# fusioninfer/fusioninfer

Hardware: NVIDIA H100
Metric: routing decisions/sec (4K-tok prompts x 1024 endpoints); achieved HBM GB/s (higher is better)
Workload: dtype u64

## Files before the change

### fusioninfer_b200/csrc/bitslice.cuh

```cuda
#pragma once
#include <stdint.h>

#include "xxh64.cuh"

namespace fi {

constexpr int NPLANES = 10;

struct BitCounter {
  uint32_t c[NPLANES];
};

FI_HD void bc_clear(BitCounter& b) {
#pragma unroll
  for (int i = 0; i < NPLANES; ++i) b.c[i] = 0;
}

template <int LVL>
FI_HD void bc_ripple(BitCounter& b, uint32_t e) {
#pragma unroll
  for (int pl = LVL; pl < NPLANES; ++pl) {
    uint32_t t = b.c[pl] & e;
    b.c[pl] ^= e;
    e = t;
// ... 27 lines not shown
      w[i] = (a & x) | (a & y) | (x & y);
    }
  }
  if (K >= 16) {
    uint32_t a = b.c[3], x = w[0], y = w[1 % K];
    b.c[3] = a ^ x ^ y;
    w[0] = (a & x) | (a & y) | (x & y);
  }
  if (K == 1) bc_ripple<0>(b, w[0]);
  if (K == 2) bc_ripple<1>(b, w[0]);
  if (K == 4) bc_ripple<2>(b, w[0]);
  if (K == 8) bc_ripple<3>(b, w[0]);
  if (K == 16) bc_ripple<4>(b, w[0]);
}

FI_HD void bc_merge(BitCounter& b, const BitCounter& o) {
  uint32_t carry = 0;
#pragma unroll
  for (int pl = 0; pl < NPLANES; ++pl) {
    uint32_t x = b.c[pl], y = o.c[pl];
    b.c[pl] = x ^ y ^ carry;
    carry = (x & y) | (x & carry) | (y & carry);
  }
}

FI_HD uint32_t bc_nonzero(const BitCounter& b) {
  uint32_t m = 0;
#pragma unroll
  for (int pl = 0; pl < NPLANES; ++pl) m |= b.c[pl];
  return m;
// ... 11 lines not shown
```

### fusioninfer_b200/csrc/engine.cu

```cuda
#include <cuda_runtime.h>
#include <unistd.h>
#include <dlfcn.h>

#include <algorithm>
#include <atomic>
#include <chrono>
#include <cmath>
#include <condition_variable>
#include <cstdio>
#include <cstdlib>
#include <cstring>
#include <functional>
#include <memory>
#include <mutex>
#include <string>
#include <thread>
#include <unordered_set>
#include <vector>

#include <sched.h>

#include "../../include/fi_epp.h"
#include "kernels.cuh"
#include "lru.h"
// ... 303 lines not shown
      }
    }
    h->ev_pool.push_back(e.a);
    h->ev_pool.push_back(e.b);
  }
  h->pending_ev.clear();
}

void free_index(IndexView& v) {
  cudaFree(v.keys);
  cudaFree(v.node_of);
  cudaFree(v.klog);
  cudaFree(v.rows);
  cudaFree(v.cnt);
  cudaFree(v.rmask);
  v.keys = nullptr;
  v.node_of = nullptr;
  v.klog = nullptr;
  v.rows = nullptr;
  v.cnt = nullptr;
  v.rmask = nullptr;
}

size_t index_bytes(uint64_t slots, uint32_t W) {
  const uint64_t total = slots + 3;
  return total * (sizeof(uint64_t) * 2 + sizeof(uint32_t) * 3 + (size_t)W * sizeof(uint32_t));
}

int clear_index(fi_epp* h, IndexView& v) {
  const uint64_t total = v.C + 3;
  FI_CUDA(cudaMemsetAsync(v.keys, 0, total * sizeof(uint64_t), h->s_index));
  FI_CUDA(cudaMemsetAsync(v.node_of, 0xFF, total * sizeof(uint32_t), h->s_index));
  FI_CUDA(cudaMemsetAsync(v.klog, 0, total * sizeof(uint64_t), h->s_index));
  FI_CUDA(cudaMemsetAsync(v.rows, 0, total * v.W * sizeof(uint32_t), h->s_index));
  FI_CUDA(cudaMemsetAsync(v.cnt, 0, total * sizeof(uint32_t), h->s_index));
  FI_CUDA(cudaMemsetAsync(v.rmask, 0, total * sizeof(uint32_t), h->s_index));
  return FI_OK;
}

int alloc_index(fi_epp* h, uint64_t slots, IndexView* out) {
  IndexView v{};
  v.C = slots;
  v.bmask = slots / BUCKET_KEYS - 1;
  v.W = h->W;
  v.logW = 0;
  while ((1u << v.logW) < v.W) ++v.logW;
  const uint64_t total = slots + 3;
  size_t free_b = 0, total_b = 0;
  if (cudaMemGetInfo(&free_b, &total_b) == cudaSuccess && index_bytes(slots, v.W) + (256ull << 20) > free_b) {
    h->err = "index of " + std::to_string(index_bytes(slots, v.W) >> 20) + " MiB does not fit in the " +
             std::to_string(free_b >> 20) + " MiB of free device memory";
    return FI_ERR_NOMEM;
  }
  cudaError_t e = cudaMalloc(&v.keys, total * sizeof(uint64_t));
  if (e == cudaSuccess) e = cudaMalloc(&v.node_of, total * sizeof(uint32_t));
  if (e == cudaSuccess) e = cudaMalloc(&v.klog, total * sizeof(uint64_t));
  if (e == cudaSuccess) e = cudaMalloc(&v.rows, total * v.W * sizeof(uint32_t));
  if (e == cudaSuccess) e = cudaMalloc(&v.cnt, total * sizeof(uint32_t));
  if (e == cudaSuccess) e = cudaMalloc(&v.rmask, total * sizeof(uint32_t));
  if (e != cudaSuccess) {
    cudaGetLastError();
    free_index(v);
    h->err = std::string("index allocation: ") + cudaGetErrorString(e);
    return e == cudaErrorMemoryAllocation ? FI_ERR_NOMEM : FI_ERR_CUDA;
  }
  int rc = clear_index(h, v);
  if (rc != FI_OK) {
    free_index(v);
    return rc;
  }
  *out = v;
  return FI_OK;
}

// ... 2308 lines not shown
  drain_profile(h);
  h->profiling = on != 0;
  return FI_OK;
}

int fi_epp_get_stats(fi_epp* h, fi_epp_stats* out) {
  if (!h || !out) return FI_ERR_INVALID;
  std::lock_guard<std::mutex> lk(h->mu);
  if (cudaSetDevice(h->cfg.device) != cudaSuccess) return fail(h, FI_ERR_CUDA, "cudaSetDevice failed");
  drain_profile(h);
  if (h->profiling) {
    FI_CUDA(cudaStreamSynchronize(h->s_main));
    unsigned long long pb[8] = {0};
    FI_CUDA(cudaMemcpy(pb, h->d_probed, sizeof(pb), cudaMemcpyDeviceToHost));
    h->stats.probed_blocks = pb[0];
    if (pb[5] && h->verbose)
      std::fprintf(stderr, "[fi_epp] match_pick phases, cycles per request over %llu requests: stage %.0f, first lookup %.0f, "
                   "chunks %.0f, score+pick %.0f\n", pb[5], (double)pb[1] / pb[5], (double)pb[2] / pb[5], (double)pb[3] / pb[5],
                   (double)pb[4] / pb[5]);
  }
  *out = h->stats;
  return FI_OK;
}

int fi_epp_reset_stats(fi_epp* h) {
  if (!h) return FI_ERR_INVALID;
  std::lock_guard<std::mutex> lk(h->mu);
  cudaSetDevice(h->cfg.device);
  drain_profile(h);
  cudaStreamSynchronize(h->s_main);
// ... 7 lines not shown
```

### fusioninfer_b200/csrc/hostcheck.cpp

```cpp
#include <cstdint>
#include <cstring>
#include <algorithm>
#include <set>
#include <unordered_map>
#include <unordered_set>
#include <vector>

#include "bitslice.cuh"
#include "lru.h"
#include "lru_batch.h"
#include "lru_plan.h"
#include "tiebreak.cuh"
#include "xxh64.cuh"

extern "C" {

uint64_t fihc_xxh64(const uint8_t* p, uint32_t len) { return fi::xxh64_bytes(p, len); }

uint32_t fihc_chain_generic(const uint8_t* p, uint64_t len, uint64_t h0, uint32_t B, uint32_t M, uint64_t* out) {
  uint64_t nb = len / B;
  if (nb > M) nb = M;
  uint64_t h = h0;
  for (uint64_t i = 0; i < nb; ++i) {
    fi::ChainMsg m{p + i * B, B, h, true};
// ... 25 lines not shown
void fihc_bitcount(const uint32_t* words, uint32_t n, uint32_t K, uint32_t* counts) {
  fi::BitCounter b;
  fi::bc_clear(b);
  for (uint32_t i = 0; i < n; i += K) {
    uint32_t w[16] = {0};
    for (uint32_t j = 0; j < K && i + j < n; ++j) w[j] = words[i + j];
    switch (K) {
      case 1: { uint32_t t[1] = {w[0]}; fi::bc_add<1>(b, t); break; }
      case 2: { uint32_t t[2] = {w[0], w[1]}; fi::bc_add<2>(b, t); break; }
      case 4: { uint32_t t[4]; std::memcpy(t, w, sizeof(t)); fi::bc_add<4>(b, t); break; }
      case 8: { uint32_t t[8]; std::memcpy(t, w, sizeof(t)); fi::bc_add<8>(b, t); break; }
      default: { uint32_t t[16]; std::memcpy(t, w, sizeof(t)); fi::bc_add<16>(b, t); break; }
    }
  }
  for (uint32_t bit = 0; bit < 32; ++bit) counts[bit] = fi::bc_get(b, bit);
}

void fihc_bitcount_merge(const uint32_t* wa, uint32_t na, const uint32_t* wb, uint32_t nb, uint32_t* counts,
                         uint32_t* nonzero) {
  fi::BitCounter a, b;
  fi::bc_clear(a);
  fi::bc_clear(b);
  for (uint32_t i = 0; i < na; ++i) { uint32_t t[1] = {wa[i]}; fi::bc_add<1>(a, t); }
  for (uint32_t i = 0; i < nb; ++i) { uint32_t t[1] = {wb[i]}; fi::bc_add<1>(b, t); }
  fi::bc_merge(a, b);
  for (uint32_t bit = 0; bit < 32; ++bit) counts[bit] = fi::bc_get(a, bit);
  *nonzero = fi::bc_nonzero(a);
}

uint32_t fihc_tie_start(uint32_t n_blocks, uint64_t first_hash, uint64_t h0, uint32_t r, uint32_t E) {
// ... 200 lines not shown
```

### fusioninfer_b200/csrc/index_kernels.cu

```cuda
#include "index_device.cuh"
#include "kernels.cuh"

namespace fi {

namespace {

__device__ uint32_t table_find_or_claim(const IndexView& ix, IndexCounters* ctr, uint64_t h, bool* claimed) {
  *claimed = false;
  uint64_t b = h & ix.bmask;
  for (uint64_t it = 0; it <= ix.bmask; ++it) {
    unsigned long long* kb = reinterpret_cast<unsigned long long*>(ix.keys + b * BUCKET_KEYS);
#pragma unroll 1
    for (int j = 0; j < BUCKET_KEYS; ++j) {
      unsigned long long k = *reinterpret_cast<volatile unsigned long long*>(kb + j);
      if (k == h) return (uint32_t)(b * BUCKET_KEYS + j);
      if (k == KEY_EMPTY) {
        unsigned long long old = atomicCAS(kb + j, (unsigned long long)KEY_EMPTY, (unsigned long long)h);
        if (old == KEY_EMPTY) {
          *claimed = true;
          return (uint32_t)(b * BUCKET_KEYS + j);
        }
        if (old == h) return (uint32_t)(b * BUCKET_KEYS + j);
      }
    }
// ... 19 lines not shown
      tot += c;
    }
    s_base = tot ? atomicAdd(counter, (unsigned long long)tot) : 0ull;
  }
  __syncthreads();
  const unsigned long long pos = flag ? s_base + s_warp[warp] + rank_in_warp : ~0ull;
  __syncthreads();
  return pos;
}

__device__ __forceinline__ uint32_t wait_node(const IndexView& ix, uint32_t slot) {
  const volatile uint32_t* p = ix.node_of + slot;
  uint32_t n;
  while ((n = *p) == NODE_INVALID) __nanosleep(20);
  return n;
}

template <bool REMOTE>
__global__ void __launch_bounds__(256) index_set_kernel(IndexView ix, IndexCounters* ctr, const fi_index_op* __restrict__ ops,
                                                        const uint64_t* __restrict__ hashes, uint64_t n, uint32_t ep_begin,
                                                        uint32_t ep_count, uint32_t rank, GossipLog log) {
  const uint32_t rbit = 1u << rank;
  const uint32_t zero_node = (uint32_t)(ix.C + 2);
  for (uint64_t base = blockIdx.x * (uint64_t)blockDim.x; base < n; base += (uint64_t)gridDim.x * blockDim.x) {
    const uint64_t i = base + threadIdx.x;
    uint64_t hsh = 0;
    bool active = false;
    uint32_t e = 0;
    if (i < n) {
      if (REMOTE) {
// ... 22 lines not shown
      } else {
        atomicExch(&ctr->overflow, 1ull);
        ix.keys[slot] = KEY_TOMB;
        __threadfence();
        *reinterpret_cast<volatile uint32_t*>(ix.node_of + slot) = zero_node;
      }
    }
    if (active && !claimed && slot != SLOT_MISS) node = wait_node(ix, slot);
    bool appear = false;
    if (active && node != NODE_INVALID && node != zero_node) {
      if (REMOTE) {
        atomicOr(ix.rmask + node, rbit);
      } else {
        const uint32_t bit = 1u << (e & 31);
        const uint32_t old = atomicOr(ix.rows + ((uint64_t)node << ix.logW) + (e >> 5), bit);
        if (!(old & bit) && atomicAdd(ix.cnt + node, 1u) == 0u) {
          atomicOr(ix.rmask + node, rbit);
          appear = true;
        }
      }
    }
    if (!REMOTE && log.n_appear) {
      const unsigned long long pos = cta_reserve(appear, log.n_appear);
      if (appear && pos < log.cap) log.appear[pos] = hsh;
    }
  }
}

__device__ uint32_t table_find_slot(const IndexView& ix, uint64_t h) {
  uint64_t b = h & ix.bmask;
// ... 46 lines not shown
    uint32_t slot = SLOT_MISS, node;
    if (key_is_special(hsh)) {
      node = (uint32_t)(ix.C + (hsh == KEY_TOMB ? 1 : 0));
    } else {
      slot = table_find_slot(ix, hsh);
      if (slot == SLOT_MISS) continue;
      node = ix.node_of[slot];
      if (node >= ix.C) continue;
    }
    if (REMOTE) {
      rank_vanished(ix, ctr, slot, node, rbit);
      continue;
    }
    const uint32_t bit = 1u << (e & 31);
    const uint32_t old = atomicAnd(ix.rows + ((uint64_t)node << ix.logW) + (e >> 5), ~bit);
    if ((old & bit) && atomicSub(ix.cnt + node, 1u) == 1u) {
      rank_vanished(ix, ctr, slot, node, rbit);
      if (log.n_vanish) {
        const unsigned long long pos = atomicAdd(log.n_vanish, 1ull);
        if (pos < log.cap) log.vanish[pos] = hsh;
      }
    }
  }
}

__global__ void __launch_bounds__(256) index_rebuild_kernel(IndexView from, IndexView to, IndexCounters* ctr) {
  for (uint64_t base = blockIdx.x * (uint64_t)blockDim.x; base < from.C; base += (uint64_t)gridDim.x * blockDim.x) {
    const uint64_t s = base + threadIdx.x;
    uint64_t h = 0;
    if (s < from.C) h = from.klog[s];
    bool claimed = false;
    uint32_t slot = SLOT_MISS;
    if (h != 0) slot = table_find_or_claim(to, ctr, h, &claimed);
    const unsigned long long d = cta_reserve(claimed, &ctr->used);
    if (claimed && d < to.C) {
      to.klog[d] = h;
      to.node_of[slot] = (uint32_t)d;
      to.cnt[d] = from.cnt[s];
      to.rmask[d] = from.rmask[s];
      const uint32_t* src = from.rows + (s << from.logW);
      uint32_t* dst = to.rows + (d << to.logW);
      for (uint32_t w = 0; w < from.W; ++w) dst[w] = src[w];
    }
  }
  if (blockIdx.x == 0 && threadIdx.x < 2) {
    const uint64_t s = from.C + threadIdx.x;
    if (from.rmask[s]) {
      to.cnt[s] = from.cnt[s];
      to.rmask[s] = from.rmask[s];
      for (uint32_t w = 0; w < from.W; ++w) to.rows[(s << to.logW) + w] = from.rows[(s << from.logW) + w];
    }
  }
}


__device__ __forceinline__ uint32_t sweep_node(const IndexView& ix, uint64_t t, uint64_t n) {
  return (uint32_t)(t < n ? t : ix.C + (t - n));
}
// ... 104 lines not shown
      if (node != SLOT_MISS) r = (ix.rows[((uint64_t)node << ix.logW) + (e >> 5)] >> (e & 31)) & 1u;
    }
    out[i] = r;
  }
}

inline unsigned grid_for(uint64_t n) {
  uint64_t g = (n + 255) / 256;
  if (g > 132ull * 16) g = 132ull * 16;
  if (g == 0) g = 1;
  return (unsigned)g;
}

}

cudaError_t launch_index_set(IndexView ix, IndexCounters* ctr, const fi_index_op* ops, uint64_t n, uint32_t ep_begin,
                             uint32_t ep_count, uint32_t rank, GossipLog log, cudaStream_t s) {
  if (n == 0) return cudaSuccess;
  index_set_kernel<false><<<grid_for(n), 256, 0, s>>>(ix, ctr, ops, nullptr, n, ep_begin, ep_count, rank, log);
  return cudaGetLastError();
}

cudaError_t launch_index_clear(IndexView ix, IndexCounters* ctr, const fi_index_op* ops, uint64_t n,
                               uint32_t ep_begin, uint32_t ep_count, uint32_t rank, GossipLog log, cudaStream_t s) {
  if (n == 0) return cudaSuccess;
  index_clear_kernel<false><<<grid_for(n), 256, 0, s>>>(ix, ctr, ops, nullptr, n, ep_begin, ep_count, rank, log, nullptr);
  return cudaGetLastError();
}

cudaError_t launch_index_clear_counted(IndexView ix, IndexCounters* ctr, const fi_index_op* ops, uint64_t cap,
                                       const unsigned long long* n_dev, uint32_t ep_begin, uint32_t ep_count, uint32_t rank,
                                       GossipLog log, cudaStream_t s) {
  if (cap == 0) return cudaSuccess;
  index_clear_kernel<false><<<grid_for(cap), 256, 0, s>>>(ix, ctr, ops, nullptr, cap, ep_begin, ep_count, rank, log, n_dev);
  return cudaGetLastError();
}

cudaError_t launch_index_remote_appear(IndexView ix, IndexCounters* ctr, const uint64_t* hashes, uint64_t n, uint32_t rank,
                                       cudaStream_t s) {
  if (n == 0) return cudaSuccess;
  index_set_kernel<true><<<grid_for(n), 256, 0, s>>>(ix, ctr, nullptr, hashes, n, 0, 0, rank, GossipLog{});
  return cudaGetLastError();
}

cudaError_t launch_index_remote_vanish(IndexView ix, IndexCounters* ctr, const uint64_t* hashes, uint64_t n, uint32_t rank,
                                       cudaStream_t s) {
  if (n == 0) return cudaSuccess;
  index_clear_kernel<true><<<grid_for(n), 256, 0, s>>>(ix, ctr, nullptr, hashes, n, 0, 0, rank, GossipLog{}, nullptr);
  return cudaGetLastError();
}
// ... 26 lines not shown
```

### fusioninfer_b200/csrc/kernels.cuh

```cuda
#pragma once
#include <cuda_runtime.h>
#include <stdint.h>

#include "../../include/fi_epp.h"

namespace fi {

constexpr uint32_t SLOT_MISS = 0xFFFFFFFFu;
constexpr uint64_t KEY_EMPTY = 0ull;
constexpr uint64_t KEY_TOMB = ~0ull;
constexpr int BUCKET_KEYS = 4;

struct IndexView {
  uint64_t* keys;
  uint32_t* node_of;
  uint64_t* klog;
  uint32_t* rows;
  uint32_t* cnt;
  uint32_t* rmask;
  uint64_t bmask;
  uint64_t C;
  uint32_t W;
  uint32_t logW;
};

struct IndexCounters {
  unsigned long long used;
  unsigned long long tombstones;
  unsigned long long overflow;
  unsigned long long pad;
};

struct GossipLog {
  unsigned long long* n_appear;
// ... 162 lines not shown
```

### fusioninfer_b200/csrc/match_kernels.cu

```cuda
#include <climits>

#include "bitslice.cuh"
#include "index_device.cuh"
#include "kernels.cuh"
#include "tiebreak.cuh"

namespace fi {

namespace {

constexpr int kWarps = 8;
#ifndef FI_MATCH_MIN_BLOCKS
#define FI_MATCH_MIN_BLOCKS 2
#endif
constexpr unsigned FULL = 0xFFFFFFFFu;

struct Best {
  double score;
  uint32_t e;
  uint32_t m;
  uint32_t k;
};

struct TieRot {
  uint32_t start;
  uint32_t E;
// ... 39 lines not shown
      else if (pr.kind[s] == FI_SCORER_LORA)
        v = lora_v;
      else if (REQ_QUEUE && pr.kind[s] == FI_SCORER_QUEUE)
        v = q_v;
      else
        v = sc_p[(uint64_t)s * Epad + e];
      total = __dadd_rn(total, __dmul_rn(v, pr.weight[s]));
    }
  }
  return total;
}

__device__ __forceinline__ void cp_async16(void* smem, const void* gmem) {
  unsigned sa = (unsigned)__cvta_generic_to_shared(smem);
  asm volatile("cp.async.cg.shared.global [%0], [%1], 16;\n" ::"r"(sa), "l"(gmem));
}
__device__ __forceinline__ void cp_async_wait_all() { asm volatile("cp.async.wait_all;\n" ::: "memory"); }
__device__ __forceinline__ void ll_store(uint64_t* p, uint32_t data, uint32_t tag) {
  asm volatile("st.relaxed.sys.global.u64 [%0], %1;\n" ::"l"(p), "l"(((uint64_t)tag << 32) | data) : "memory");
}
__device__ __forceinline__ uint64_t ll_load(const uint64_t* p) {
  uint64_t v;
  asm volatile("ld.relaxed.sys.global.u64 %0, [%1];\n" : "=l"(v) : "l"(p) : "memory");
  return v;
}
constexpr long long kPollTimeoutCycles = 20000000000ll;
__device__ __forceinline__ bool pd_prefill_runs(uint32_t dec_endpoint, uint32_t dec_match, uint32_t n, uint64_t len,
                                                double threshold) {
  double hit = (dec_endpoint != FI_NO_ENDPOINT && n) ? __ddiv_rn((double)dec_match, (double)n) : 0.0;
  double miss_bytes = __dmul_rn(__dsub_rn(1.0, hit), (double)len);
// ... 10 lines not shown
    out[2 % VEC] = v.z;
    out[3 % VEC] = v.w;
  } else if (VEC == 2) {
    uint2 v = make_uint2(0, 0);
    if (ok) v = __ldg(reinterpret_cast<const uint2*>(p));
    out[0] = v.x;
    out[1 % VEC] = v.y;
  } else {
    out[0] = ok ? __ldg(p) : 0u;
  }
}

constexpr int kSpecTries = 4;
constexpr int kSpecChunks = 8;

__device__ __forceinline__ uint32_t resolve_request_nodes(const IndexView& ix, const uint64_t* __restrict__ s_chain,
                                                          uint32_t* __restrict__ s_node, uint32_t n, int lane, bool have_first,
                                                          uint32_t first_node) {
  uint32_t pos = 0;
  for (int tries = 0; pos < n; ++tries) {
    if (tries < kSpecTries) {
      uint32_t nf = SLOT_MISS;
      if (tries == 0 && have_first) {
        nf = first_node;
      } else {
        if (lane == 0) nf = index_find(ix, s_chain[pos]);
        nf = __shfl_sync(FULL, nf, 0);
      }
      if (nf == SLOT_MISS) return pos;
      if (lane == 0) s_node[pos] = nf;
      uint32_t fail = n;
      if (nf >= ix.C) {
        fail = pos + 1;
      } else {
        for (uint32_t i0 = pos + 1; i0 < n && fail == n; i0 += 32 * kSpecChunks) {
          uint64_t hk[kSpecChunks], kk[kSpecChunks];
#pragma unroll
          for (int c = 0; c < kSpecChunks; ++c) {
            const uint32_t idx = i0 + 32 * c + lane;
            hk[c] = 0;
            kk[c] = 1;
            if (idx < n) {
              hk[c] = s_chain[idx];
              const uint64_t cand = (uint64_t)nf + (idx - pos);
              if (cand < ix.C) kk[c] = __ldg(ix.klog + cand);
            }
          }
#pragma unroll
          for (int c = 0; c < kSpecChunks; ++c) {
            const uint32_t idx = i0 + 32 * c + lane;
            if (fail != n || i0 + 32 * c >= n) break;
            const bool ok = idx < n && kk[c] == hk[c] && !key_is_special(hk[c]);
            const unsigned bad = __ballot_sync(FULL, idx < n && !ok);
            const uint32_t upto = bad ? (uint32_t)(__ffs(bad) - 1) : 32u;
            if ((uint32_t)lane < upto && idx < n) s_node[idx] = nf + (idx - pos);
            if (bad) fail = i0 + 32 * c + upto;
          }
        }
      }
      pos = fail;
    } else {
      const uint32_t ia = pos + lane, ib = pos + 32 + lane;
      uint32_t na = SLOT_MISS, nb = SLOT_MISS;
      if (ia < n) na = index_find_lazy(ix, s_chain[ia]);
      if (ib < n) nb = index_find_lazy(ix, s_chain[ib]);
      const unsigned ma = __ballot_sync(FULL, ia < n && na == SLOT_MISS);
      const unsigned mb = __ballot_sync(FULL, ib < n && nb == SLOT_MISS);
      const uint32_t upto = ma ? (uint32_t)(__ffs(ma) - 1) : (mb ? 32u + (uint32_t)(__ffs(mb) - 1) : 64u);
      if ((uint32_t)lane < upto && ia < n) s_node[ia] = na;
      if ((uint32_t)lane + 32 < upto && ib < n) s_node[ib] = nb;
      if (ma || mb) return pos + upto;
      pos = pos + 64 < n ? pos + 64 : n;
    }
  }
  return n;
}

__device__ __forceinline__ uint32_t take_ticket(uint32_t* counter, uint32_t opaque_zero) {
  uint32_t t;
  asm volatile("atom.relaxed.gpu.global.add.u32 %0, [%1], 1;\n" : "=r"(t) : "l"(counter + opaque_zero) : "memory");
  return t;
}

template <int VEC, int G, bool SUBSET>
__device__ __forceinline__ void ranked_profile(const MatchParams& p, uint32_t pi, const BitCounter (&cnt)[VEC],
                                               const uint32_t (&sub)[VEC], const TieRot& tr, uint32_t n, uint32_t r,
                                               int lane, int t, int g, uint32_t& dec_e, uint32_t& dec_m) {
  const ProfileDev& pr = p.st.prof[pi];
  const double* sc_p = p.st.sc + (uint64_t)pi * FI_EPP_MAX_SCORERS * p.st.Epad;
  const bool lora = p.st.has_lora != 0;
// ... 105 lines not shown
__global__ void __launch_bounds__(kWarps * 32, (VEC >= 4 || RANKED ? FI_MATCH_MIN_BLOCKS : FI_MATCH_MIN_BLOCKS + 1))
    match_pick_kernel(const MatchParams p) {
  constexpr int G = 32 / LPR;
#ifndef FI_MATCH_BATCH
#define FI_MATCH_BATCH 16
#endif
  constexpr int BATCH_MAX = (LPM || VEC >= 4) ? 8 : FI_MATCH_BATCH;
  constexpr int BATCH = LPR < BATCH_MAX ? LPR : BATCH_MAX;
  extern __shared__ __align__(16) uint64_t s_mem[];
  const int warp = threadIdx.x >> 5;
  const int lane = threadIdx.x & 31;
  const int t = lane % LPR;
  const int g = lane / LPR;
  uint64_t* const s_chain_base = s_mem + (size_t)(2 * warp) * p.MP;
  uint32_t* s_node = reinterpret_cast<uint32_t*>(s_mem + (size_t)2 * kWarps * p.MP) + (size_t)warp * p.MP;
  const IndexView ix = p.ix;
  const uint32_t P = p.st.n_profiles;
  const char* row_base = reinterpret_cast<const char*>(ix.rows + t * VEC);
  const uint32_t row_bytes = 4u << ix.logW;
  const uint32_t zero_slot = (uint32_t)(ix.C + 2);

  const uint32_t row_units = p.MP / 2;
  auto stage = [&](uint32_t rr, uint64_t* dst) {
    const uint64_t* crow = p.chain + (uint64_t)rr * p.MP;
    for (uint32_t u = lane; u < row_units; u += 32) cp_async16(dst + 2 * u, crow + 2 * u);
  };
  uint32_t r_next = 0;
  if (lane == 0) r_next = take_ticket(p.work_counter, threadIdx.x & p.lane_zero);
  r_next = __shfl_sync(FULL, r_next, 0);
  int buf = 0;
  if (r_next < p.R) stage(r_next, s_chain_base);
  bool pf_ok = false;
  uint64_t pf_h = 0, pf_key = 0;
  uint32_t pf_node = 0;
  for (;;) {
    const uint32_t r = r_next;
    if (r >= p.R) break;
    if (lane == 0) r_next = take_ticket(p.work_counter, threadIdx.x & p.lane_zero);
    const uint32_t n = p.nblocks[r];
    uint32_t sub[VEC];
#pragma unroll
    for (int x = 0; x < VEC; ++x) {
      sub[x] = 0u;
      if constexpr (SUBSET) {
        const uint32_t wi = t * VEC + x;
        if (wi < p.sub_pitch) sub[x] = __ldg(p.subsets + (uint64_t)r * p.sub_pitch + wi);
      }
    }
    uint64_t* s_chain = s_chain_base + (size_t)buf * p.MP;
#ifdef FI_MATCH_TIMING
    const long long tm0 = clock64();
#endif
    cp_async_wait_all();
    __syncwarp();
    bool have_first = false;
    uint32_t first_node = SLOT_MISS;
    if (pf_ok && n) {
      const unsigned hit = __ballot_sync(FULL, lane < BUCKET_KEYS && pf_key == pf_h);
      const unsigned emp = __ballot_sync(FULL, lane < BUCKET_KEYS && pf_key == KEY_EMPTY);
      if (hit) {
        first_node = __shfl_sync(FULL, pf_node, __ffs(hit) - 1);
        have_first = true;
      } else if (emp) {
        have_first = true;
      }
    }

#ifdef FI_MATCH_TIMING
    const long long tm1 = clock64();
#endif
    BitCounter cnt[VEC];
    uint32_t alive[VEC];
#pragma unroll
    for (int x = 0; x < VEC; ++x) {
      bc_clear(cnt[x]);
      alive[x] = 0xFFFFFFFFu;
    }
    uint32_t matched_rows = 0;
    bool real_miss = false;

    const uint32_t m_rows = resolve_request_nodes(ix, s_chain, s_node, n, lane, have_first, first_node);
    real_miss = m_rows < n;
    __syncwarp();
    r_next = __shfl_sync(FULL, r_next, 0);
    pf_ok = false;
    if (r_next < p.R) {
      stage(r_next, s_chain_base + (size_t)(buf ^ 1) * p.MP);
      pf_h = __ldg(p.chain + (uint64_t)r_next * p.MP);
    }
#ifdef FI_MATCH_TIMING
    const long long tm2 = clock64();
#endif
#pragma unroll 1
    for (uint32_t b0 = 0; b0 < m_rows; b0 += BATCH * G) {
      uint32_t w[VEC][BATCH];
#pragma unroll
      for (int qi = 0; qi < BATCH; ++qi) {
        const uint32_t j = b0 + qi * G + g;
        const uint32_t sn = j < m_rows ? s_node[j] : zero_slot;
        uint32_t tmp[VEC];
        load_row_words<VEC>(reinterpret_cast<const uint32_t*>(row_base + (uint64_t)sn * row_bytes), true, tmp);
#pragma unroll
        for (int x = 0; x < VEC; ++x) w[x][qi] = tmp[x];
      }
      if (LPM) {
#pragma unroll
        for (int qi = 0; qi < BATCH; ++qi) {
#pragma unroll
          for (int x = 0; x < VEC; ++x) {
            uint32_t v = w[x][qi];
            if (G > 1) {
#pragma unroll
              for (int d = 1; d < G; d <<= 1) {
                const uint32_t o = __shfl_up_sync(FULL, v, d * LPR);
                if (g >= d) v &= o;
              }
              v &= alive[x];
              alive[x] = __shfl_sync(FULL, v, (G - 1) * LPR + t);
            } else {
              v &= alive[x];
              alive[x] = v;
            }
            w[x][qi] = v;
          }
        }
      }
#pragma unroll
      for (int x = 0; x < VEC; ++x) {
        uint32_t any = 0;
#pragma unroll
        for (int qi = 0; qi < BATCH; ++qi) any |= w[x][qi];
        if (__any_sync(FULL, any != 0)) bc_add<BATCH>(cnt[x], w[x]);
      }
      matched_rows = min(m_rows, b0 + BATCH * G);
      if (LPM) {
        bool any = false;
#pragma unroll
        for (int x = 0; x < VEC; ++x) any |= alive[x] != 0;
        if (!__ballot_sync(FULL, any)) break;
      }
    }

    if (r_next < p.R && !key_is_special(pf_h)) {
      pf_ok = true;
      if (lane < BUCKET_KEYS) {
        const uint64_t slot0 = (pf_h & ix.bmask) * BUCKET_KEYS + lane;
        pf_key = __ldg(ix.keys + slot0);
        pf_node = __ldg(ix.node_of + slot0);
      }
    }
#ifdef FI_MATCH_TIMING
    const long long tm3 = clock64();
#endif
    const bool nothing = matched_rows == 0;
    if (G > 1 && !nothing) {
#pragma unroll
      for (int x = 0; x < VEC; ++x) {
#pragma unroll
        for (int d = LPR; d < 32; d <<= 1) {
          BitCounter o;
#pragma unroll
          for (int pl = 0; pl < NPLANES; ++pl) o.c[pl] = __shfl_xor_sync(FULL, cnt[x].c[pl], d);
          bc_merge(cnt[x], o);
// ... 123 lines not shown
      if (p.apply_pd) {
        const uint64_t len = p.offsets[r + 1] - p.offsets[r];
        if (!pd_prefill_runs(dec_e, dec_m, n, len, p.pd_threshold)) {
          fi_pick pk;
          pk.endpoint = FI_NO_ENDPOINT;
          pk.match_blocks = 0;
          pk.n_blocks = (uint16_t)n;
          pk.score = 0.0;
          if constexpr (RANKED) {
            for (uint32_t j = 0; j < p.k; ++j) p.out[((uint64_t)r * P + p.pd_prefill) * p.k + j] = pk;
          } else {
            p.out[(uint64_t)r * P + p.pd_prefill] = pk;
          }
        }
      }
      if (p.probed_blocks) atomicAdd(p.probed_blocks, (unsigned long long)(matched_rows + (real_miss ? 1 : 0)));
#ifdef FI_MATCH_TIMING
      if (p.probed_blocks) {
        const long long tm4 = clock64();
        atomicAdd(p.probed_blocks + 1, (unsigned long long)(tm1 - tm0));
        atomicAdd(p.probed_blocks + 2, (unsigned long long)(tm2 - tm1));
        atomicAdd(p.probed_blocks + 3, (unsigned long long)(tm3 - tm2));
        atomicAdd(p.probed_blocks + 4, (unsigned long long)(tm4 - tm3));
        atomicAdd(p.probed_blocks + 5, 1ull);
      }
#endif
    }
    buf ^= 1;
    __syncwarp();
  }
}
// ... 154 lines not shown
    __syncthreads();
    const double zbest = s_best;
    for (uint32_t e = tid; e < st.Epad; e += blockDim.x) {
      bool ok;
      const double tot = zero_total(e, &ok, false);
      const unsigned word = __ballot_sync(FULL, ok && tot == zbest);
      if (lane == 0) ztie[(uint64_t)pi * W + e / 32] = word;
    }
    __syncthreads();
  }
}

template <int LPR, int VEC, bool LPM, bool LORA, bool RANKED, bool SUBSET = false>
cudaError_t launch_match_variant(const MatchParams& p, int sm_count, cudaStream_t s) {
  const auto kern = match_pick_kernel<LPR, VEC, LPM, LORA, RANKED, SUBSET>;
  const size_t smem = (size_t)kWarps * p.MP * (2 * sizeof(uint64_t) + sizeof(uint32_t));
  static size_t cached_smem_dev[64];
  static int cached_per_sm_dev[64];
  int dev = 0;
  cudaError_t e = cudaGetDevice(&dev);
  if (e != cudaSuccess) return e;
  dev &= 63;
  size_t& cached_smem = cached_smem_dev[dev];
  int& cached_per_sm = cached_per_sm_dev[dev];
  if (cached_smem != smem + 1) {
    if (smem > 48 * 1024) {
      e = cudaFuncSetAttribute(kern, cudaFuncAttributeMaxDynamicSharedMemorySize, (int)smem);
      if (e != cudaSuccess) return e;
    }
    int per_sm = 0;
    e = cudaOccupancyMaxActiveBlocksPerMultiprocessor(&per_sm, kern, kWarps * 32, smem);
// ... 62 lines not shown
```

Before: 90.29 million.

## Skip identical consecutive index rows using a same-as-previous bitmap in match

Adds a per-slot bitmap recording whether an index row equals the previous slot's row, maintained by dirty-list fixup kernels after index set/clear and carried through rebuild. The match kernel compresses each request's matched chain into run heads and adds each distinct row once with a run-length bit-sliced add, instead of reading every row. The aim is to cut HBM row traffic for long prefix chains. The first-bucket prefetch also moves to shared memory through cp.async. In exchange, index updates get extra atomics and a fixup kernel launch, and the match path gets more branching and shared-memory bookkeeping.

```diff
diff --git a/fusioninfer_b200/csrc/bitslice.cuh b/fusioninfer_b200/csrc/bitslice.cuh
--- a/fusioninfer_b200/csrc/bitslice.cuh
+++ b/fusioninfer_b200/csrc/bitslice.cuh
@@ -65,6 +65,16 @@
   if (K == 16) bc_ripple<4>(b, w[0]);
 }
 
+FI_HD void bc_add_run(BitCounter& b, uint32_t L, uint32_t w) {
+  uint32_t carry = 0;
+#pragma unroll
+  for (int pl = 0; pl < NPLANES; ++pl) {
+    const uint32_t x = b.c[pl], y = w & (0u - ((L >> pl) & 1u));
+    b.c[pl] = x ^ y ^ carry;
+    carry = (x & y) | (x & carry) | (y & carry);
+  }
+}
+
 FI_HD void bc_merge(BitCounter& b, const BitCounter& o) {
   uint32_t carry = 0;
 #pragma unroll
diff --git a/fusioninfer_b200/csrc/engine.cu b/fusioninfer_b200/csrc/engine.cu
--- a/fusioninfer_b200/csrc/engine.cu
+++ b/fusioninfer_b200/csrc/engine.cu
@@ -341,17 +341,28 @@
   cudaFree(v.rows);
   cudaFree(v.cnt);
   cudaFree(v.rmask);
+  cudaFree(v.same);
+  cudaFree(v.dirty);
+  cudaFree(v.n_dirty);
   v.keys = nullptr;
   v.node_of = nullptr;
   v.klog = nullptr;
   v.rows = nullptr;
   v.cnt = nullptr;
   v.rmask = nullptr;
-}
+  v.same = nullptr;
+  v.dirty = nullptr;
+  v.n_dirty = nullptr;
+}
+
+constexpr uint64_t kDirtyCap = kOpChunk;
+
+uint64_t same_words(uint64_t slots) { return slots / 32 + 1; }
 
 size_t index_bytes(uint64_t slots, uint32_t W) {
   const uint64_t total = slots + 3;
-  return total * (sizeof(uint64_t) * 2 + sizeof(uint32_t) * 3 + (size_t)W * sizeof(uint32_t));
+  return total * (sizeof(uint64_t) * 2 + sizeof(uint32_t) * 3 + (size_t)W * sizeof(uint32_t)) +
+         same_words(slots) * sizeof(uint32_t) + kDirtyCap * sizeof(uint32_t) + sizeof(unsigned long long);
 }
 
 int clear_index(fi_epp* h, IndexView& v) {
@@ -362,6 +373,8 @@
   FI_CUDA(cudaMemsetAsync(v.rows, 0, total * v.W * sizeof(uint32_t), h->s_index));
   FI_CUDA(cudaMemsetAsync(v.cnt, 0, total * sizeof(uint32_t), h->s_index));
   FI_CUDA(cudaMemsetAsync(v.rmask, 0, total * sizeof(uint32_t), h->s_index));
+  FI_CUDA(cudaMemsetAsync(v.same, 0, same_words(v.C) * sizeof(uint32_t), h->s_index));
+  FI_CUDA(cudaMemsetAsync(v.n_dirty, 0, sizeof(unsigned long long), h->s_index));
   return FI_OK;
 }
 
@@ -385,6 +398,10 @@
   if (e == cudaSuccess) e = cudaMalloc(&v.rows, total * v.W * sizeof(uint32_t));
   if (e == cudaSuccess) e = cudaMalloc(&v.cnt, total * sizeof(uint32_t));
   if (e == cudaSuccess) e = cudaMalloc(&v.rmask, total * sizeof(uint32_t));
+  if (e == cudaSuccess) e = cudaMalloc(&v.same, same_words(slots) * sizeof(uint32_t));
+  if (e == cudaSuccess) e = cudaMalloc(&v.dirty, kDirtyCap * sizeof(uint32_t));
+  if (e == cudaSuccess) e = cudaMalloc(&v.n_dirty, sizeof(unsigned long long));
+  v.dirty_cap = kDirtyCap;
   if (e != cudaSuccess) {
     cudaGetLastError();
     free_index(v);
@@ -2723,6 +2740,8 @@
     unsigned long long pb[8] = {0};
     FI_CUDA(cudaMemcpy(pb, h->d_probed, sizeof(pb), cudaMemcpyDeviceToHost));
     h->stats.probed_blocks = pb[0];
+    if (h->verbose && pb[0])
+      std::fprintf(stderr, "[fi_epp] match_pick rows read %llu for %llu blocks probed\n", pb[6], pb[0]);
     if (pb[5] && h->verbose)
       std::fprintf(stderr, "[fi_epp] match_pick phases, cycles per request over %llu requests: stage %.0f, first lookup %.0f, "
                    "chunks %.0f, score+pick %.0f\n", pb[5], (double)pb[1] / pb[5], (double)pb[2] / pb[5], (double)pb[3] / pb[5],
diff --git a/fusioninfer_b200/csrc/hostcheck.cpp b/fusioninfer_b200/csrc/hostcheck.cpp
--- a/fusioninfer_b200/csrc/hostcheck.cpp
+++ b/fusioninfer_b200/csrc/hostcheck.cpp
@@ -63,6 +63,17 @@
     }
   }
   for (uint32_t bit = 0; bit < 32; ++bit) counts[bit] = fi::bc_get(b, bit);
+}
+
+void fihc_bitcount_run(const uint32_t* planes, uint32_t L, uint32_t w, uint32_t* run_out, uint32_t* rep_out) {
+  fi::BitCounter a, b;
+  for (int pl = 0; pl < fi::NPLANES; ++pl) a.c[pl] = b.c[pl] = planes[pl];
+  fi::bc_add_run(a, L, w);
+  for (uint32_t i = 0; i < L; ++i) { uint32_t t[1] = {w}; fi::bc_add<1>(b, t); }
+  for (int pl = 0; pl < fi::NPLANES; ++pl) {
+    run_out[pl] = a.c[pl];
+    rep_out[pl] = b.c[pl];
+  }
 }
 
 void fihc_bitcount_merge(const uint32_t* wa, uint32_t na, const uint32_t* wb, uint32_t nb, uint32_t* counts,
diff --git a/fusioninfer_b200/csrc/index_kernels.cu b/fusioninfer_b200/csrc/index_kernels.cu
--- a/fusioninfer_b200/csrc/index_kernels.cu
+++ b/fusioninfer_b200/csrc/index_kernels.cu
@@ -57,6 +57,72 @@
   uint32_t n;
   while ((n = *p) == NODE_INVALID) __nanosleep(20);
   return n;
+}
+
+__device__ __forceinline__ void mark_dirty(const IndexView& ix, uint32_t node) {
+  if (node >= ix.C) return;
+  const unsigned long long pos = atomicAdd(ix.n_dirty, 1ull);
+  if (pos < ix.dirty_cap) ix.dirty[pos] = node;
+}
+
+__device__ __forceinline__ bool rows_equal(const IndexView& ix, uint64_t a, uint64_t b) {
+  const uint32_t* ra = ix.rows + (a << ix.logW);
+  const uint32_t* rb = ix.rows + (b << ix.logW);
+  if (ix.W >= 4) {
+    uint32_t diff = 0;
+    for (uint32_t w = 0; w < ix.W; w += 4) {
+      const uint4 x = *reinterpret_cast<const uint4*>(ra + w), y = *reinterpret_cast<const uint4*>(rb + w);
+      diff |= (x.x ^ y.x) | (x.y ^ y.y) | (x.z ^ y.z) | (x.w ^ y.w);
+    }
+    return diff == 0;
+  }
+  for (uint32_t w = 0; w < ix.W; ++w)
+    if (ra[w] != rb[w]) return false;
+  return true;
+}
+
+__device__ __forceinline__ bool same_bit_of(const IndexView& ix, uint64_t n, uint64_t used) {
+  return n >= 1 && n < used && rows_equal(ix, n, n - 1);
+}
+
+__device__ __forceinline__ void same_sweep(const IndexView& ix, uint64_t used) {
+  const uint32_t lane = threadIdx.x & 31;
+  const uint64_t words = (used + 31) / 32;
+  const uint64_t nwarps = (uint64_t)gridDim.x * (blockDim.x / 32);
+  for (uint64_t wi = (blockIdx.x * (uint64_t)blockDim.x + threadIdx.x) / 32; wi < words; wi += nwarps) {
+    uint32_t word = 0;
+    for (uint32_t i = 0; i < 32; ++i) {
+      const uint64_t n = wi * 32 + i;
+      if (n >= used) break;
+      if (n == 0) continue;
+      uint32_t diff = 0;
+      for (uint32_t w = lane; w < ix.W; w += 32)
+        diff |= ix.rows[(n << ix.logW) + w] ^ ix.rows[((n - 1) << ix.logW) + w];
+      if (!__any_sync(0xFFFFFFFFu, diff != 0)) word |= 1u << i;
+    }
+    if (lane == 0) ix.same[wi] = word;
+  }
+}
+
+__device__ __forceinline__ void set_same_bit(const IndexView& ix, uint64_t n, bool v) {
+  const uint32_t m = 1u << (n & 31);
+  if (v) atomicOr(ix.same + (n >> 5), m);
+  else atomicAnd(ix.same + (n >> 5), ~m);
+}
+
+__global__ void __launch_bounds__(256) index_same_fixup_kernel(IndexView ix, IndexCounters* ctr) {
+  const unsigned long long nd = *ix.n_dirty;
+  const uint64_t used_ctr = *reinterpret_cast<volatile unsigned long long*>(&ctr->used);
+  const uint64_t used = used_ctr < ix.C ? used_ctr : ix.C;
+  if (nd > ix.dirty_cap) {
+    same_sweep(ix, used);
+    return;
+  }
+  for (uint64_t i = blockIdx.x * (uint64_t)blockDim.x + threadIdx.x; i < nd; i += (uint64_t)gridDim.x * blockDim.x) {
+    const uint64_t n = ix.dirty[i];
+    set_same_bit(ix, n, same_bit_of(ix, n, used));
+    if (n + 1 < ix.C) set_same_bit(ix, n + 1, same_bit_of(ix, n + 1, used));
+  }
 }
 
 template <bool REMOTE>
@@ -109,6 +175,7 @@
       } else {
         const uint32_t bit = 1u << (e & 31);
         const uint32_t old = atomicOr(ix.rows + ((uint64_t)node << ix.logW) + (e >> 5), bit);
+        if (!(old & bit)) mark_dirty(ix, node);
         if (!(old & bit) && atomicAdd(ix.cnt + node, 1u) == 0u) {
           atomicOr(ix.rmask + node, rbit);
           appear = true;
@@ -185,6 +252,7 @@
     }
     const uint32_t bit = 1u << (e & 31);
     const uint32_t old = atomicAnd(ix.rows + ((uint64_t)node << ix.logW) + (e >> 5), ~bit);
+    if (old & bit) mark_dirty(ix, node);
     if ((old & bit) && atomicSub(ix.cnt + node, 1u) == 1u) {
       rank_vanished(ix, ctr, slot, node, rbit);
       if (log.n_vanish) {
@@ -196,6 +264,7 @@
 }
 
 __global__ void __launch_bounds__(256) index_rebuild_kernel(IndexView from, IndexView to, IndexCounters* ctr) {
+  __shared__ uint8_t s_claimed[256];
   for (uint64_t base = blockIdx.x * (uint64_t)blockDim.x; base < from.C; base += (uint64_t)gridDim.x * blockDim.x) {
     const uint64_t s = base + threadIdx.x;
     uint64_t h = 0;
@@ -203,7 +272,10 @@
     bool claimed = false;
     uint32_t slot = SLOT_MISS;
     if (h != 0) slot = table_find_or_claim(to, ctr, h, &claimed);
+    s_claimed[threadIdx.x] = claimed;
     const unsigned long long d = cta_reserve(claimed, &ctr->used);
+    if (claimed && d < to.C && threadIdx.x > 0 && s_claimed[threadIdx.x - 1] && ((from.same[s >> 5] >> (s & 31)) & 1u))
+      atomicOr(to.same + (d >> 5), 1u << (d & 31));
     if (claimed && d < to.C) {
       to.klog[d] = h;
       to.node_of[slot] = (uint32_t)d;
@@ -213,6 +285,7 @@
       uint32_t* dst = to.rows + (d << to.logW);
       for (uint32_t w = 0; w < from.W; ++w) dst[w] = src[w];
     }
+    __syncthreads();
   }
   if (blockIdx.x == 0 && threadIdx.x < 2) {
     const uint64_t s = from.C + threadIdx.x;
@@ -347,18 +420,27 @@
 
 }
 
+static cudaError_t launch_same_fixup(IndexView ix, IndexCounters* ctr, uint64_t n, cudaStream_t s) {
+  cudaError_t e = cudaGetLastError();
+  if (e != cudaSuccess) return e;
+  index_same_fixup_kernel<<<grid_for(n < ix.dirty_cap ? n : ix.dirty_cap), 256, 0, s>>>(ix, ctr);
+  e = cudaGetLastError();
+  if (e != cudaSuccess) return e;
+  return cudaMemsetAsync(ix.n_dirty, 0, sizeof(unsigned long long), s);
+}
+
 cudaError_t launch_index_set(IndexView ix, IndexCounters* ctr, const fi_index_op* ops, uint64_t n, uint32_t ep_begin,
                              uint32_t ep_count, uint32_t rank, GossipLog log, cudaStream_t s) {
   if (n == 0) return cudaSuccess;
   index_set_kernel<false><<<grid_for(n), 256, 0, s>>>(ix, ctr, ops, nullptr, n, ep_begin, ep_count, rank, log);
-  return cudaGetLastError();
+  return launch_same_fixup(ix, ctr, n, s);
 }
 
 cudaError_t launch_index_clear(IndexView ix, IndexCounters* ctr, const fi_index_op* ops, uint64_t n,
                                uint32_t ep_begin, uint32_t ep_count, uint32_t rank, GossipLog log, cudaStream_t s) {
   if (n == 0) return cudaSuccess;
   index_clear_kernel<false><<<grid_for(n), 256, 0, s>>>(ix, ctr, ops, nullptr, n, ep_begin, ep_count, rank, log, nullptr);
-  return cudaGetLastError();
+  return launch_same_fixup(ix, ctr, n, s);
 }
 
 cudaError_t launch_index_clear_counted(IndexView ix, IndexCounters* ctr, const fi_index_op* ops, uint64_t cap,
@@ -366,7 +448,7 @@
                                        GossipLog log, cudaStream_t s) {
   if (cap == 0) return cudaSuccess;
   index_clear_kernel<false><<<grid_for(cap), 256, 0, s>>>(ix, ctr, ops, nullptr, cap, ep_begin, ep_count, rank, log, n_dev);
-  return cudaGetLastError();
+  return launch_same_fixup(ix, ctr, cap, s);
 }
 
 cudaError_t launch_index_remote_appear(IndexView ix, IndexCounters* ctr, const uint64_t* hashes, uint64_t n, uint32_t rank,
diff --git a/fusioninfer_b200/csrc/kernels.cuh b/fusioninfer_b200/csrc/kernels.cuh
--- a/fusioninfer_b200/csrc/kernels.cuh
+++ b/fusioninfer_b200/csrc/kernels.cuh
@@ -18,6 +18,10 @@
   uint32_t* rows;
   uint32_t* cnt;
   uint32_t* rmask;
+  uint32_t* same;
+  uint32_t* dirty;
+  unsigned long long* n_dirty;
+  uint64_t dirty_cap;
   uint64_t bmask;
   uint64_t C;
   uint32_t W;
diff --git a/fusioninfer_b200/csrc/match_kernels.cu b/fusioninfer_b200/csrc/match_kernels.cu
--- a/fusioninfer_b200/csrc/match_kernels.cu
+++ b/fusioninfer_b200/csrc/match_kernels.cu
@@ -10,6 +10,7 @@
 namespace {
 
 constexpr int kWarps = 8;
+constexpr int kPfWords = 8;
 #ifndef FI_MATCH_MIN_BLOCKS
 #define FI_MATCH_MIN_BLOCKS 2
 #endif
@@ -79,6 +80,14 @@
 __device__ __forceinline__ void cp_async16(void* smem, const void* gmem) {
   unsigned sa = (unsigned)__cvta_generic_to_shared(smem);
   asm volatile("cp.async.cg.shared.global [%0], [%1], 16;\n" ::"r"(sa), "l"(gmem));
+}
+__device__ __forceinline__ void cp_async8(void* smem, const void* gmem) {
+  unsigned sa = (unsigned)__cvta_generic_to_shared(smem);
+  asm volatile("cp.async.ca.shared.global [%0], [%1], 8;\n" ::"r"(sa), "l"(gmem));
+}
+__device__ __forceinline__ void cp_async4(void* smem, const void* gmem) {
+  unsigned sa = (unsigned)__cvta_generic_to_shared(smem);
+  asm volatile("cp.async.ca.shared.global [%0], [%1], 4;\n" ::"r"(sa), "l"(gmem));
 }
 __device__ __forceinline__ void cp_async_wait_all() { asm volatile("cp.async.wait_all;\n" ::: "memory"); }
 __device__ __forceinline__ void ll_store(uint64_t* p, uint32_t data, uint32_t tag) {
@@ -119,10 +128,12 @@
 constexpr int kSpecTries = 4;
 constexpr int kSpecChunks = 8;
 
-__device__ __forceinline__ uint32_t resolve_request_nodes(const IndexView& ix, const uint64_t* __restrict__ s_chain,
-                                                          uint32_t* __restrict__ s_node, uint32_t n, int lane, bool have_first,
-                                                          uint32_t first_node) {
+__device__ __forceinline__ uint32_t resolve_request_nodes(const IndexView& ix, const uint64_t* s_chain,
+                                                          uint32_t* __restrict__ s_node, uint32_t* s_hidx, uint32_t n,
+                                                          int lane, bool have_first, uint32_t first_node, uint32_t& H) {
+  const unsigned lt = (1u << lane) - 1u;
   uint32_t pos = 0;
+  H = 0;
   for (int tries = 0; pos < n; ++tries) {
     if (tries < kSpecTries) {
       uint32_t nf = SLOT_MISS;
@@ -132,14 +143,24 @@
         if (lane == 0) nf = index_find(ix, s_chain[pos]);
         nf = __shfl_sync(FULL, nf, 0);
       }
-      if (nf == SLOT_MISS) return pos;
-      if (lane == 0) s_node[pos] = nf;
+      if (nf == SLOT_MISS) break;
+      __syncwarp();
+      if (lane == 0) {
+        s_node[H] = nf;
+        if (H) s_hidx[H] = pos;
+      }
+      ++H;
       uint32_t fail = n;
       if (nf >= ix.C) {
         fail = pos + 1;
       } else {
         for (uint32_t i0 = pos + 1; i0 < n && fail == n; i0 += 32 * kSpecChunks) {
           uint64_t hk[kSpecChunks], kk[kSpecChunks];
+          uint32_t swl = 0;
+          if (lane < 2 * kSpecChunks) {
+            const uint64_t wi = (((uint64_t)nf + (i0 + 32 * (lane & 7) - pos)) >> 5) + (lane >> 3);
+            if (wi <= (ix.C >> 5)) swl = __ldg(ix.same + wi);
+          }
 #pragma unroll
           for (int c = 0; c < kSpecChunks; ++c) {
             const uint32_t idx = i0 + 32 * c + lane;
@@ -148,9 +169,12 @@
             if (idx < n) {
               hk[c] = s_chain[idx];
               const uint64_t cand = (uint64_t)nf + (idx - pos);
-              if (cand < ix.C) kk[c] = __ldg(ix.klog + cand);
+              if (cand < ix.C) {
+                kk[c] = __ldg(ix.klog + cand);
+              }
             }
           }
+          __syncwarp();
 #pragma unroll
           for (int c = 0; c < kSpecChunks; ++c) {
             const uint32_t idx = i0 + 32 * c + lane;
@@ -158,7 +182,18 @@
             const bool ok = idx < n && kk[c] == hk[c] && !key_is_special(hk[c]);
             const unsigned bad = __ballot_sync(FULL, idx < n && !ok);
             const uint32_t upto = bad ? (uint32_t)(__ffs(bad) - 1) : 32u;
-            if ((uint32_t)lane < upto && idx < n) s_node[idx] = nf + (idx - pos);
+            const uint32_t node = nf + (idx - pos);
+            const bool valid = (uint32_t)lane < upto && idx < n;
+            const uint32_t lo = __shfl_sync(FULL, swl, c), hi = __shfl_sync(FULL, swl, kSpecChunks + c);
+            const uint32_t off = ((nf + (i0 + 32 * c - pos)) & 31u) + (uint32_t)lane;
+            const uint32_t same = off < 32 ? (lo >> off) & 1u : (hi >> (off - 32)) & 1u;
+            const unsigned heads = __ballot_sync(FULL, valid && !same);
+            if (valid && ((heads >> lane) & 1u)) {
+              const uint32_t k = H + __popc(heads & lt);
+              s_node[k] = node;
+              s_hidx[k] = idx;
+            }
+            H += __popc(heads);
             if (bad) fail = i0 + 32 * c + upto;
           }
         }
@@ -172,13 +207,23 @@
       const unsigned ma = __ballot_sync(FULL, ia < n && na == SLOT_MISS);
       const unsigned mb = __ballot_sync(FULL, ib < n && nb == SLOT_MISS);
       const uint32_t upto = ma ? (uint32_t)(__ffs(ma) - 1) : (mb ? 32u + (uint32_t)(__ffs(mb) - 1) : 64u);
-      if ((uint32_t)lane < upto && ia < n) s_node[ia] = na;
-      if ((uint32_t)lane + 32 < upto && ib < n) s_node[ib] = nb;
-      if (ma || mb) return pos + upto;
-      pos = pos + 64 < n ? pos + 64 : n;
-    }
-  }
-  return n;
+      const uint32_t got = min(upto, n - pos);
+      __syncwarp();
+      if ((uint32_t)lane < got) {
+        s_node[H + lane] = na;
+        if (H + lane) s_hidx[H + lane] = ia;
+      }
+      if ((uint32_t)lane + 32 < got) {
+        s_node[H + 32 + lane] = nb;
+        s_hidx[H + 32 + lane] = ib;
+      }
+      H += got;
+      pos += got;
+      if (ma || mb) break;
+    }
+  }
+  if (H && lane == 0) s_hidx[H] = pos;
+  return pos;
 }
 
 __device__ __forceinline__ uint32_t take_ticket(uint32_t* counter, uint32_t opaque_zero) {
@@ -314,6 +359,8 @@
   const int g = lane / LPR;
   uint64_t* const s_chain_base = s_mem + (size_t)(2 * warp) * p.MP;
   uint32_t* s_node = reinterpret_cast<uint32_t*>(s_mem + (size_t)2 * kWarps * p.MP) + (size_t)warp * p.MP;
+  uint64_t* const s_pf_key = s_mem + (size_t)2 * kWarps * p.MP + (size_t)kWarps * p.MP / 2 + (size_t)warp * kPfWords;
+  uint32_t* const s_pf_node = reinterpret_cast<uint32_t*>(s_pf_key + BUCKET_KEYS);
   const IndexView ix = p.ix;
   const uint32_t P = p.st.n_profiles;
   const char* row_base = reinterpret_cast<const char*>(ix.rows + t * VEC);
@@ -331,8 +378,7 @@
   int buf = 0;
   if (r_next < p.R) stage(r_next, s_chain_base);
   bool pf_ok = false;
-  uint64_t pf_h = 0, pf_key = 0;
-  uint32_t pf_node = 0;
+  uint64_t pf_h = 0;
   for (;;) {
     const uint32_t r = r_next;
     if (r >= p.R) break;
@@ -356,10 +402,12 @@
     bool have_first = false;
     uint32_t first_node = SLOT_MISS;
     if (pf_ok && n) {
-      const unsigned hit = __ballot_sync(FULL, lane < BUCKET_KEYS && pf_key == pf_h);
+      const uint64_t h_first = s_chain[0];
+      const uint64_t pf_key = lane < BUCKET_KEYS ? s_pf_key[lane] : 0ull;
+      const unsigned hit = __ballot_sync(FULL, lane < BUCKET_KEYS && pf_key == h_first);
       const unsigned emp = __ballot_sync(FULL, lane < BUCKET_KEYS && pf_key == KEY_EMPTY);
       if (hit) {
-        first_node = __shfl_sync(FULL, pf_node, __ffs(hit) - 1);
+        first_node = s_pf_node[__ffs(hit) - 1];
         have_first = true;
       } else if (emp) {
         have_first = true;
@@ -376,10 +424,11 @@
       bc_clear(cnt[x]);
       alive[x] = 0xFFFFFFFFu;
     }
-    uint32_t matched_rows = 0;
     bool real_miss = false;
 
-    const uint32_t m_rows = resolve_request_nodes(ix, s_chain, s_node, n, lane, have_first, first_node);
+    uint32_t* const s_hidx = reinterpret_cast<uint32_t*>(s_chain) + 1;
+    uint32_t H;
+    const uint32_t m_rows = resolve_request_nodes(ix, s_chain, s_node, s_hidx, n, lane, have_first, first_node, H);
     real_miss = m_rows < n;
     __syncwarp();
     r_next = __shfl_sync(FULL, r_next, 0);
@@ -391,48 +440,69 @@
 #ifdef FI_MATCH_TIMING
     const long long tm2 = clock64();
 #endif
+    auto hstart = [&](uint32_t k) -> uint32_t { return k ? s_hidx[k] : 0u; };
+    uint32_t heads_read = 0;
 #pragma unroll 1
-    for (uint32_t b0 = 0; b0 < m_rows; b0 += BATCH * G) {
+    for (uint32_t b0 = 0; b0 < H; b0 += BATCH * G) {
       uint32_t w[VEC][BATCH];
 #pragma unroll
       for (int qi = 0; qi < BATCH; ++qi) {
         const uint32_t j = b0 + qi * G + g;
-        const uint32_t sn = j < m_rows ? s_node[j] : zero_slot;
+        const uint32_t sn = j < H ? s_node[j] : zero_slot;
         uint32_t tmp[VEC];
         load_row_words<VEC>(reinterpret_cast<const uint32_t*>(row_base + (uint64_t)sn * row_bytes), true, tmp);
 #pragma unroll
         for (int x = 0; x < VEC; ++x) w[x][qi] = tmp[x];
       }
-      if (LPM) {
-#pragma unroll
-        for (int qi = 0; qi < BATCH; ++qi) {
+      const uint32_t hend = min(H, b0 + BATCH * G);
+      if (s_hidx[hend] - hstart(b0) == hend - b0) {
+        if (LPM) {
+#pragma unroll
+          for (int qi = 0; qi < BATCH; ++qi) {
+#pragma unroll
+            for (int x = 0; x < VEC; ++x) {
+              uint32_t v = w[x][qi];
+              if (G > 1) {
+#pragma unroll
+                for (int d = 1; d < G; d <<= 1) {
+                  const uint32_t o = __shfl_up_sync(FULL, v, d * LPR);
+                  if (g >= d) v &= o;
+                }
+                v &= alive[x];
+                alive[x] = __shfl_sync(FULL, v, (G - 1) * LPR + t);
+              } else {
+                v &= alive[x];
+                alive[x] = v;
+              }
+              w[x][qi] = v;
+            }
+          }
+        }
+#pragma unroll
+        for (int x = 0; x < VEC; ++x) {
+          uint32_t any = 0;
+#pragma unroll
+          for (int qi = 0; qi < BATCH; ++qi) any |= w[x][qi];
+          if (__any_sync(FULL, any != 0)) bc_add<BATCH>(cnt[x], w[x]);
+        }
+      } else {
+#pragma unroll 1
+        for (uint32_t j = b0 + (LPM ? 0u : (uint32_t)g); j < hend; j += (LPM ? 1u : (uint32_t)G)) {
+          uint32_t row[VEC];
+          load_row_words<VEC>(reinterpret_cast<const uint32_t*>(row_base + (uint64_t)s_node[j] * row_bytes), true, row);
+          const uint32_t L = (LPM && j % G != (uint32_t)g) ? 0u : s_hidx[j + 1] - hstart(j);
 #pragma unroll
           for (int x = 0; x < VEC; ++x) {
-            uint32_t v = w[x][qi];
-            if (G > 1) {
-#pragma unroll
-              for (int d = 1; d < G; d <<= 1) {
-                const uint32_t o = __shfl_up_sync(FULL, v, d * LPR);
-                if (g >= d) v &= o;
-              }
-              v &= alive[x];
-              alive[x] = __shfl_sync(FULL, v, (G - 1) * LPR + t);
-            } else {
+            uint32_t v = row[x];
+            if (LPM) {
               v &= alive[x];
               alive[x] = v;
             }
-            w[x][qi] = v;
-          }
-        }
-      }
-#pragma unroll
-      for (int x = 0; x < VEC; ++x) {
-        uint32_t any = 0;
-#pragma unroll
-        for (int qi = 0; qi < BATCH; ++qi) any |= w[x][qi];
-        if (__any_sync(FULL, any != 0)) bc_add<BATCH>(cnt[x], w[x]);
-      }
-      matched_rows = min(m_rows, b0 + BATCH * G);
+            bc_add_run(cnt[x], L, v);
+          }
+        }
+      }
+      heads_read = hend;
       if (LPM) {
         bool any = false;
 #pragma unroll
@@ -440,13 +510,14 @@
         if (!__ballot_sync(FULL, any)) break;
       }
     }
+    const uint32_t matched_rows = heads_read ? s_hidx[heads_read] : 0u;
 
     if (r_next < p.R && !key_is_special(pf_h)) {
       pf_ok = true;
       if (lane < BUCKET_KEYS) {
         const uint64_t slot0 = (pf_h & ix.bmask) * BUCKET_KEYS + lane;
-        pf_key = __ldg(ix.keys + slot0);
-        pf_node = __ldg(ix.node_of + slot0);
+        cp_async8(s_pf_key + lane, ix.keys + slot0);
+        cp_async4(s_pf_node + lane, ix.node_of + slot0);
       }
     }
 #ifdef FI_MATCH_TIMING
@@ -600,7 +671,10 @@
           }
         }
       }
-      if (p.probed_blocks) atomicAdd(p.probed_blocks, (unsigned long long)(matched_rows + (real_miss ? 1 : 0)));
+      if (p.probed_blocks) {
+        atomicAdd(p.probed_blocks, (unsigned long long)(matched_rows + (real_miss ? 1 : 0)));
+        atomicAdd(p.probed_blocks + 6, (unsigned long long)heads_read);
+      }
 #ifdef FI_MATCH_TIMING
       if (p.probed_blocks) {
         const long long tm4 = clock64();
@@ -785,7 +859,7 @@
 template <int LPR, int VEC, bool LPM, bool LORA, bool RANKED, bool SUBSET = false>
 cudaError_t launch_match_variant(const MatchParams& p, int sm_count, cudaStream_t s) {
   const auto kern = match_pick_kernel<LPR, VEC, LPM, LORA, RANKED, SUBSET>;
-  const size_t smem = (size_t)kWarps * p.MP * (2 * sizeof(uint64_t) + sizeof(uint32_t));
+  const size_t smem = (size_t)kWarps * p.MP * (2 * sizeof(uint64_t) + sizeof(uint32_t)) + (size_t)kWarps * kPfWords * sizeof(uint64_t);
   static size_t cached_smem_dev[64];
   static int cached_per_sm_dev[64];
   int dev = 0;
```

After: 94.63 million, median of 6. +4.8%, better.
